# SpursLipu/YOLOv3v4-ModelCompression-MultidatasetTraining-Multibackbone

Measured on AMD Instinct MI355X. Metric: images/sec YOLOv3-608 train fp16, higher is better.
Workload: dtype f16; 1 GPU; YOLOv3 Darknet-53 608 COCO (80 classes) fp16 training step, batch 64/GPU: train-mode forward (batch-stat BN) + compute_loss + backward + nesterov SGD, single GPU; global_batch=64, parallelism=dp1

## Files before the change

include/yolo_hip.h:

```cpp
#ifndef YOLO_HIP_H
#define YOLO_HIP_H

#include <stdint.h>

#ifdef __cplusplus
extern "C" {
#endif

#define YH_ABI_VERSION 2

enum { YH_F16 = 0, YH_F32 = 1, YH_I8 = 2 };

enum { YH_ACT_LINEAR = 0, YH_ACT_LEAKY = 1, YH_ACT_RELU = 2, YH_ACT_RELU6 = 3, YH_ACT_HSWISH = 4, YH_ACT_MISH = 5 };

enum {
    YH_OK = 0,
    YH_EINVAL = -1,
    YH_EALIGN = -2,
    YH_EUNSUPPORTED = -3,
    YH_ENOMEM = -4,
    YH_ERANGE = -5
};

int yh_abi_version(void);
// ... 24 lines not shown
    float acc_scale;
    float out_scale;
    int32_t y_h, y_w;
    int32_t y_off_h, y_off_w;
    float* stats_ws;
    int64_t stats_ws_floats;
    float q_rx, q_ra, q_scale_x, q_scale_a, q_inv_scale_sum;
    const void* bwd_z;
    const float* bwd_gamma;
    const float* bwd_beta;
    const float* bwd_mean;
    const float* bwd_invstd;
    int32_t bwd_ldz, bwd_act;
    float bwd_slope;
    int32_t bwd_reserved;
} yh_conv_desc;
int64_t yh_conv2d_stats_rows(const yh_conv_desc* d);
int64_t yh_conv2d_bwd_stats_rows(const yh_conv_desc* d);

int yh_conv2d_fwd(const yh_conv_desc* d, void* stream);
int yh_qconv_pack_weights(const float* q_weight, float w_scale, const int32_t* cin_map, int cout, int cin, int kh, int kw,
                          int cin_k, int m_pad, void* packed, void* stream);
int yh_conv2d_tile(const yh_conv_desc* d);

typedef struct yh_stem_desc {
    const float* x;
    const float* w;
    const float* bias;
    void* y;
    int32_t n, cin, h, w_in, ho, wo, cout, cout_pad, kh, kw, stride, pad, ldy, act;
    float slope;
    int32_t dtype;
    float out_scale;
// ... 356 lines not shown
```

yolov3v4-modelcompression-multidatasettraining-multibackbone_amd/csrc/conv_igemm.h:

```cpp
#pragma once
#include <type_traits>

#include "common.h"

namespace yh {

struct ConvArgs {
    const void* x;
    const void* w;
    const float* bias;
    const void* res;
    void* y;
    int N, H, W, Cin, Ho, Wo, Cout, R, S, stride, pad;
    int ldx, ldr, ldy;
    int cin_k;
    int ktot;
    long P;
    int m_tiles, p_tiles;
    int m_pad;
    float acc_scale, out_scale, inv_out_scale;
    int act;
    float slope;
    int ups;
    float* stats_part;
    int y_h, y_w, y_off_h, y_off_w;
    float q_rx, q_ra, q_scale_x, q_scale_a, q_inv_scale_sum;
    int no_lds_store;
    int hpp_stagger;
    const void* bz;
    const float *bgamma, *bbeta, *bmean, *binvstd;
    int ldbz, bact;
    float bslope;
};

template <int CTRL> __device__ __forceinline__ float dpp_shr_add(float v) {
    const int t = __builtin_amdgcn_update_dpp(0, __builtin_bit_cast(int, v), CTRL, 0xf, 0xf, true);
    return v + __builtin_bit_cast(float, t);
}
__device__ __forceinline__ float row16_sum(float v) {
    v = dpp_shr_add<0x111>(v);
    v = dpp_shr_add<0x112>(v);
    v = dpp_shr_add<0x114>(v);
    v = dpp_shr_add<0x118>(v);
    return v;
}

template <int N, typename F> __device__ __forceinline__ void static_for(F&& f) {
// ... 422 lines not shown
                if (a.ups == 2) {
                    store4<OutT>(dst + a.ldy, v[0], v[1], v[2], v[3]);
                    store4<OutT>(dst + (long)c.wo2 * a.ldy, v[0], v[1], v[2], v[3]);
                    store4<OutT>(dst + (long)(c.wo2 + 1) * a.ldy, v[0], v[1], v[2], v[3]);
                }
            }
        });
    });
}

int launch_k64_tile(const ConvArgs& a, int tile, int dtype, int out_f32, hipStream_t stream);
int launch_pointwise_tile(const ConvArgs& a, int dtype, int out_f32, hipStream_t stream);
int launch_stream3_tile(const ConvArgs& a, int dtype, hipStream_t stream);
long stream3_stats_rows(long P, int cout);
int launch_pwl_tile(const ConvArgs& a, int dtype, hipStream_t stream);
bool pwl_supported(int dtype, int out_f32, int cin, int cin_k, int cout, long P, int ldx, int ldy, int ldr, const void* x, const void* y,
                   const void* res, bool stats, bool bwd);
long pwl_stats_rows(long P, int cout, bool bwd = false);
int launch_hpp_tile(const ConvArgs& a, int dtype, hipStream_t stream);
bool hpp_geometry(int W, int cin_k, int bk, int* rows_hp, int* lb, int* hbufs, size_t* lds);

}
```

yolov3v4-modelcompression-multidatasettraining-multibackbone_amd/csrc/conv_igemm.hip:

```cpp
#include "conv_igemm.h"

namespace yh {

template <typename T, int TM, int TN, int KU> struct MmaStep;

template <int TM, int TN, int KU> struct MmaStep<f16, TM, TN, KU> {
    static __device__ __forceinline__ void run(const u32x4* As, const u32x4* Bs, int BM, int BN, int arow, int brow,
                                               int lane, f32x4 (&acc)[TM][TN]) {
        const int r = lane & 15;
#pragma unroll
        for (int h = 0; h < KU / 4; ++h) {
            const int u = h * 4 + (lane >> 4);
            f16x8 a[TM], b[TN];
#pragma unroll
            for (int i = 0; i < TM; ++i) {
                u32x4 v = As[u * BM + arow + i * 16 + r];
                a[i] = *reinterpret_cast<f16x8*>(&v);
            }
#pragma unroll
            for (int j = 0; j < TN; ++j) {
                u32x4 v = Bs[u * BN + brow + j * 16 + r];
                b[j] = *reinterpret_cast<f16x8*>(&v);
            }
#pragma unroll
// ... 880 lines not shown

static bool pwl_desc_supported(const yh_conv_desc* d) {
    if (d->kh != 1 || d->kw != 1 || d->stride != 1 || d->pad != 0 || d->ups != 1) return false;
    if (d->act != YH_ACT_LINEAR && d->act != YH_ACT_LEAKY && d->act != YH_ACT_MISH) return false;
    const bool bwd = d->bwd_z != nullptr;
    if (bwd && (d->act != YH_ACT_LINEAR || (d->bwd_act != YH_ACT_LEAKY && d->bwd_act != YH_ACT_MISH))) return false;
    return yh::pwl_supported(d->dtype, d->out_f32, d->cin, d->cin_k, d->cout, (long)d->n * d->ho * d->wo, d->ldx, d->ldy, d->ldr, d->x, d->y,
                             d->res, !bwd && d->stats_ws != nullptr, bwd);
}
static bool pick_pwl_tile(const yh_conv_desc* d) {
    static const bool off = getenv("YH_NO_PWL") != nullptr;
    static const long min_px = [] { const char* e = getenv("YH_PWL_MIN_PIXELS"); return e ? atol(e) : 262144L; }();
    return !off && pwl_desc_supported(d) && (long)d->n * d->ho * d->wo >= min_px;
}

extern "C" int yh_conv2d_tile(const yh_conv_desc* d) {
    if (!d) return YH_EINVAL;
    if (d->tile != 0) return d->tile;
    if (pick_pointwise_tile(d)) return 71;
    if (pick_pwl_tile(d)) return 73;
    if (pick_stream3_tile(d)) return 72;
    if (pick_hpp_tile(d)) return 43;
    if (pick_halo_tile(d)) return 41;
    if (const int pp = pick_pp_tile(d)) return pp;
    const int t = yh::pick_tile(d->cout, (long)d->n * d->ho * d->wo, d->cin_k, d->dtype == YH_F16 ? 8 : 4, d->kh * d->kw);
    if (d->ups == 2 && (t == 21 || t == 26 || t == 27 || t == 25)) {
        if (d->dtype == YH_F16) return 24;
        if (d->dtype == YH_I8) return 25;
    }
    if (d->dtype == YH_I8 && (t == 21 || t == 27) && (long)d->cin_k * d->kh * d->kw <= 256) return 25;
    return (d->dtype == YH_I8 && t == 3) ? 24 : t;
}
// ... 94 lines not shown
    a.P = (long)d->n * d->ho * d->wo;
    a.m_tiles = a.p_tiles = 0;
    a.m_pad = d->m_pad;
    a.acc_scale = d->acc_scale; a.out_scale = d->out_scale; a.inv_out_scale = d->out_scale > 0.f ? 1.f / d->out_scale : 0.f;
    a.act = d->act; a.slope = d->slope; a.ups = d->ups;
    a.y_h = d->y_h; a.y_w = d->y_w; a.y_off_h = d->y_off_h; a.y_off_w = d->y_off_w;
    a.q_rx = d->q_rx; a.q_ra = d->q_ra; a.q_scale_x = d->q_scale_x; a.q_scale_a = d->q_scale_a; a.q_inv_scale_sum = d->q_inv_scale_sum;
    if (d->dtype == YH_I8 && d->res) qadd_pow2_args(a);
    a.no_lds_store = getenv("YH_PW_DIRECT") != nullptr;
    a.hpp_stagger = 0;
    a.stats_part = nullptr;
    a.bz = nullptr;
    a.bgamma = a.bbeta = a.bmean = a.binvstd = nullptr;
    a.ldbz = a.bact = 0;
    a.bslope = 0.f;
    if (d->bwd_z) {
        const int64_t rows = yh_conv2d_bwd_stats_rows(d);
        if (rows <= 0) return YH_EUNSUPPORTED;
        if (!d->stats_ws || d->stats_ws_floats < rows * 2 * d->cout) return YH_EINVAL;
        a.stats_part = d->stats_ws;
        a.bz = d->bwd_z; a.ldbz = d->bwd_ldz; a.bact = d->bwd_act; a.bslope = d->bwd_slope;
        a.bgamma = d->bwd_gamma; a.bbeta = d->bwd_beta; a.bmean = d->bwd_mean; a.binvstd = d->bwd_invstd;
        return launch_pwl_tile(a, d->dtype, (hipStream_t)stream);
    }
    if (d->stats_ws) {
        if (d->ups != 1 || d->res || d->dtype == YH_I8 || (d->tile >= 40 && d->tile < 50 && d->tile != 43)) return YH_EINVAL;
        const int64_t rows = yh_conv2d_stats_rows(d);
        if (rows <= 0 || d->stats_ws_floats < rows * 2 * d->cout) return YH_EINVAL;
        a.stats_part = d->stats_ws;
    }
// ... 28 lines not shown
```

yolov3v4-modelcompression-multidatasettraining-multibackbone_amd/csrc/conv_pw_lds.hip:

```cpp
#include "conv_igemm.h"

namespace yh {

template <typename T> struct PwlMma;
template <> struct PwlMma<f16> {
    typedef f16x8 frag_t;
    typedef f32x4 acc_t;
    static __device__ __forceinline__ acc_t mma(const frag_t& a, const frag_t& b, const acc_t& c) {
        return __builtin_amdgcn_mfma_f32_16x16x32_f16(a, b, c, 0, 0, 0);
    }
};
template <> struct PwlMma<int8_t> {
    typedef i32x4 frag_t;
    typedef i32x4 acc_t;
    static __device__ __forceinline__ acc_t mma(const frag_t& a, const frag_t& b, const acc_t& c) {
        return __builtin_amdgcn_mfma_i32_16x16x64_i8(a, b, c, 0, 0, 0);
    }
};

template <typename T, int MT, int KS, int MS, int ACT, int MODE>
__global__ __launch_bounds__(512, 2) void conv1x1_lds_kernel(const ConvArgs a, const int nblocks) {
    typedef typename PwlMma<T>::frag_t frag_t;
    typedef typename PwlMma<T>::acc_t acc_t;
    static_assert(sizeof(T) == 2 || MODE == 0, "int8: plain mode only");
    constexpr bool RES = MODE == 1 || MODE == 3, BWD = MODE == 3 || MODE == 4;
    constexpr int CACT = BWD ? YH_ACT_LINEAR : ACT;
    constexpr int ES = sizeof(T), VEC = 16 / ES, KB = 4 * VEC;
    constexpr int NW = 8, TN = 2, BP = TN * 16;
    constexpr int ROWB = MT * 16 * ES;
    constexpr int PITCH = ROWB + 16;
    constexpr int UNITS = ROWB / 16;
    constexpr int RPI = 64 / UNITS;
    constexpr int NPASS = BP / RPI;
    constexpr int W_BYTES = MS * MT * KS * 1024;
    constexpr int BIAS_BYTES = MS * MT * 16 * 4;
    extern __shared__ __attribute__((aligned(16))) unsigned char pl_smem[];
    unsigned char* const wl = pl_smem;
    float* const bl = reinterpret_cast<float*>(pl_smem + W_BYTES);
    const int tid = threadIdx.x, lane = tid & 63;
    const int wave = __builtin_amdgcn_readfirstlane(tid >> 6);
    unsigned char* const tile = pl_smem + W_BYTES + BIAS_BYTES + wave * (BP * PITCH);
    const int pc = lane & 15, kq = lane >> 4, mq = kq << 2;
    const T* const xg = reinterpret_cast<const T*>(a.x);
    const T* const rg = reinterpret_cast<const T*>(a.res);
    T* const yg = reinterpret_cast<T*>(a.y);

    {
        const T* const wg = reinterpret_cast<const T*>(a.w);
        for (int f = wave; f < MS * MT * KS; f += NW) {
            const int rgp = f / KS, k = f - rgp * KS;
            const u32x4 v = *reinterpret_cast<const u32x4*>(wg + (long)(rgp * 16 + pc) * a.cin_k + k * KB + kq * VEC);
            *reinterpret_cast<u32x4*>(wl + (f * 64 + lane) * 16) = v;
        }
        for (int m = tid; m < MS * MT * 16; m += NW * 64) bl[m] = m < a.Cout ? a.bias[m] : 0.f;
    }
    __syncthreads();

    const int half = wave % MS;
    const int stream = (blockIdx.x * NW + wave) / MS, nstreams = gridDim.x * NW / MS;
    const int ch0 = half * MT * 16;
    const unsigned char* const wl_h = wl + half * (MT * KS * 1024) + lane * 16;
    const float* const bl_h = bl + ch0 + mq;

    const int cu = lane % UNITS, rr = lane / UNITS;
    float s1[8], s2[8];
#pragma unroll
    for (int e = 0; e < 8; ++e) s1[e] = s2[e] = 0.f;
    float pg[8], pb[8], pm[8], pi[8];
    const T* const zg = reinterpret_cast<const T*>(a.bz);
    if constexpr (BWD) {
#pragma unroll
        for (int e = 0; e < 8; ++e) {
            const int c = ch0 + cu * 8 + e;
            pg[e] = a.bgamma[c];
            pb[e] = a.bbeta[c];
            pm[e] = a.bmean[c];
            pi[e] = a.binvstd[c];
        }
    }

    frag_t fb[TN][KS];
    u32x4 rv[NPASS];
    u32x4 zv[BWD ? NPASS : 1];
    auto load_z = [&](int blk) {
#pragma unroll
        for (int q = 0; q < (BWD ? NPASS : 0); ++q) {
            long p = (long)blk * BP + rr + q * RPI;
            p = p < a.P ? p : a.P - 1;
            zv[q] = *reinterpret_cast<const u32x4*>(zg + p * a.ldbz + ch0 + cu * VEC);
        }
    };
    auto load_b = [&](int blk, int k) {
#pragma unroll
        for (int j = 0; j < TN; ++j) {
            long p = (long)blk * BP + j * 16 + pc;
            p = p < a.P ? p : a.P - 1;
            fb[j][k] = *reinterpret_cast<const frag_t*>(xg + p * a.ldx + k * KB + kq * VEC);
        }
    };
    auto load_res = [&](int blk) {
#pragma unroll
        for (int q = 0; q < NPASS; ++q) {
            long p = (long)blk * BP + rr + q * RPI;
            p = p < a.P ? p : a.P - 1;
            rv[q] = *reinterpret_cast<const u32x4*>(rg + p * a.ldr + ch0 + cu * VEC);
        }
    };

    int blk = stream;
    if (blk < nblocks) {
#pragma unroll
        for (int k = 0; k < KS; ++k) load_b(blk, k);
        if constexpr (RES) load_res(blk);
    }
    for (; blk < nblocks; blk += nstreams) {
        const int nb = blk + nstreams < nblocks ? blk + nstreams : blk;
        if constexpr (BWD) load_z(blk);
        if constexpr (RES) {
#pragma unroll
            for (int q = 0; q < NPASS; ++q) *reinterpret_cast<u32x4*>(tile + (rr + q * RPI) * PITCH + cu * 16) = rv[q];
        }
        acc_t acc[MT][TN];
#pragma unroll
        for (int i = 0; i < MT; ++i)
#pragma unroll
            for (int j = 0; j < TN; ++j) acc[i][j] = acc_t{0, 0, 0, 0};
#pragma unroll
        for (int k = 0; k < KS; ++k) {
            frag_t wa[MT];
#pragma unroll
            for (int i = 0; i < MT; ++i) wa[i] = *reinterpret_cast<const frag_t*>(wl_h + (i * KS + k) * 1024);
#pragma unroll
            for (int i = 0; i < MT; ++i)
#pragma unroll
                for (int j = 0; j < TN; ++j) acc[i][j] = PwlMma<T>::mma(wa[i], fb[j][k], acc[i][j]);
            load_b(nb, k);
        }
        if constexpr (RES) load_res(nb);
        __builtin_amdgcn_wave_barrier();
#pragma unroll
        for (int i = 0; i < MT; ++i) {
            const f32x4 bv = *reinterpret_cast<const f32x4*>(bl_h + i * 16);
#pragma unroll
            for (int j = 0; j < TN; ++j) {
                T* const cell = reinterpret_cast<T*>(tile + (j * 16 + pc) * PITCH) + i * 16 + mq;
                float v[4];
                if constexpr (sizeof(T) == 1) {
                    quantize4<CACT>(acc[i][j], bv, a, v);
                } else {
#pragma unroll
                    for (int e = 0; e < 4; ++e) v[e] = activate_t<CACT, T>(acc[i][j][e] + bv[e], a.slope);
// ... 42 lines not shown
        for (int e = 0; e < 8; ++e)
#pragma unroll
            for (int m = UNITS; m < 64; m <<= 1) {
                s1[e] += __shfl_xor(s1[e], m);
                s2[e] += __shfl_xor(s2[e], m);
            }
        if (lane < UNITS) {
            float* const row = a.stats_part + (long)stream * 2 * a.Cout + ch0 + cu * 8;
#pragma unroll
            for (int e = 0; e < 8; ++e) {
                row[e] = s1[e];
                row[a.Cout + e] = s2[e];
            }
        }
    }
}

static bool pwl_shape(int cin_k, int cout, int kb, int* mt, int* ks, int* ms, bool bwd = false) {
    if (cin_k % kb || cout % 16 || cout < 32 || cout > 256 || cin_k < kb || cin_k > 8 * kb) return false;
    *ms = bwd ? cout / 64 : (cout > 128 ? 2 : 1);
    if (bwd && (cout % 64 || *ms < 1)) return false;
    if (cout % (16 * *ms)) return false;
    *mt = cout / (16 * *ms);
    *ks = cin_k / kb;
    if (*mt > 8 || (*mt != 2 && *mt != 4 && *mt != 8) || (*ks != 1 && *ks != 2 && *ks != 4 && *ks != 8)) return false;
    return (long)cout * cin_k * (kb == 32 ? 2 : 1) <= 64 * 1024;
}

static int pwl_ms(int cout, bool bwd) { return bwd ? cout / 64 : (cout > 128 ? 2 : 1); }

// ... 39 lines not shown
    return (long)pwl_grid(P, ms, &nblocks) * 8 / ms;
}

template <typename T, int MT, int KS, int MS, int ACT> static int launch_pwl_mode(const ConvArgs& a, hipStream_t s) {
    int nblocks;
    const int grid = pwl_grid(a.P, MS, &nblocks);
    const size_t lds = (size_t)MS * MT * KS * 1024 + (size_t)MS * MT * 16 * 4 + (size_t)8 * 32 * (MT * 16 * sizeof(T) + 16);
#define YH_PWL_GO(MODE)                                                                                       \
    do {                                                                                                      \
        auto kern = conv1x1_lds_kernel<T, MT, KS, MS, ACT, MODE>;                                             \
        const hipError_t e = ensure_dynamic_lds(reinterpret_cast<const void*>(kern), lds);                    \
        if (e != hipSuccess) return (int)e;                                                                   \
        hipLaunchKernelGGL(kern, dim3(grid), dim3(512), lds, s, a, nblocks);                                  \
    } while (0)
    if constexpr (sizeof(T) == 1) {
        if (a.stats_part || a.res || a.bz) return YH_EUNSUPPORTED;
        YH_PWL_GO(0);
    } else {
        if (a.bz) {
            if constexpr ((ACT == YH_ACT_LEAKY || ACT == YH_ACT_MISH) && MT == 4 && ((KS == 1 && MS == 1) || (KS == 2 && MS == 2) || (KS == 4 && MS == 4))) {
                if (!a.stats_part) return YH_EINVAL;
                if (a.res) YH_PWL_GO(3);
                else YH_PWL_GO(4);
            } else {
                return YH_EUNSUPPORTED;
            }
        } else if (a.stats_part) YH_PWL_GO(2);
        else if (a.res) YH_PWL_GO(1);
        else YH_PWL_GO(0);
    }
#undef YH_PWL_GO
    return check_launch();
}

template <typename T, int MT, int KS, int MS> static int launch_pwl_act(const ConvArgs& a, hipStream_t s) {
    switch (a.bz ? a.bact : a.act) {
        case YH_ACT_LINEAR: return launch_pwl_mode<T, MT, KS, MS, YH_ACT_LINEAR>(a, s);
        case YH_ACT_LEAKY: return launch_pwl_mode<T, MT, KS, MS, YH_ACT_LEAKY>(a, s);
        case YH_ACT_MISH: return launch_pwl_mode<T, MT, KS, MS, YH_ACT_MISH>(a, s);
        default: return YH_EUNSUPPORTED;
    }
}

int launch_pwl_tile(const ConvArgs& a, int dtype, hipStream_t s) {
    int mt, ks, ms;
    if (!pwl_shape(a.cin_k, a.Cout, dtype == YH_I8 ? 64 : 32, &mt, &ks, &ms, a.bz != nullptr)) return YH_EUNSUPPORTED;
#define YH_PWL_CASE(T, M, K, S2) if (mt == M && ks == K && ms == S2) return launch_pwl_act<T, M, K, S2>(a, s)
    if (dtype == YH_I8) {
        YH_PWL_CASE(int8_t, 8, 4, 1);
        YH_PWL_CASE(int8_t, 4, 2, 1);
        YH_PWL_CASE(int8_t, 8, 2, 1);
        YH_PWL_CASE(int8_t, 4, 1, 1);
        YH_PWL_CASE(int8_t, 8, 4, 2);
        YH_PWL_CASE(int8_t, 8, 2, 2);
        return YH_EUNSUPPORTED;
    }
    if (dtype != YH_F16) return YH_EUNSUPPORTED;
    YH_PWL_CASE(f16, 2, 2, 1);
    YH_PWL_CASE(f16, 4, 1, 1);
    YH_PWL_CASE(f16, 4, 4, 1);
    YH_PWL_CASE(f16, 8, 2, 1);
    YH_PWL_CASE(f16, 8, 8, 1);
    YH_PWL_CASE(f16, 8, 4, 2);
    YH_PWL_CASE(f16, 8, 4, 1);
    YH_PWL_CASE(f16, 4, 2, 1);
    YH_PWL_CASE(f16, 4, 2, 2);
    YH_PWL_CASE(f16, 4, 4, 4);
#undef YH_PWL_CASE
    return YH_EUNSUPPORTED;
}

}
// ... 1 lines not shown
```

yolov3v4-modelcompression-multidatasettraining-multibackbone_amd/engine/hiplib.py:

```python
import ctypes as C
import os

_HERE = os.path.dirname(os.path.abspath(__file__))
LIB_PATH = os.environ.get('YOLO_HIP_LIB') or os.path.join(os.path.dirname(_HERE), 'libyolo_hip.so')

YH_F16, YH_F32, YH_I8 = 0, 1, 2
ACT_CODES = {'linear': 0, 'leaky': 1, 'relu': 2, 'relu6': 3, 'h_swish': 4, 'mish': 5}
OP_CONV, OP_STEM, OP_POOL, OP_COPY, OP_ADD, OP_DECODE, OP_DW, OP_SE, OP_QCOPY, OP_QPOOL, OP_QADD = 1, 2, 3, 4, 5, 6, 7, 8, 9, 10, 11

_i32, _f32, _vp, _i64 = C.c_int32, C.c_float, C.c_void_p, C.c_int64


class ConvDesc(C.Structure):
    _fields_ = [('x', _vp), ('w', _vp), ('bias', _vp), ('res', _vp), ('y', _vp),
                ('n', _i32), ('h', _i32), ('w_in', _i32), ('cin', _i32),
                ('ho', _i32), ('wo', _i32), ('cout', _i32),
                ('kh', _i32), ('kw', _i32), ('stride', _i32), ('pad', _i32),
                ('ldx', _i32), ('ldr', _i32), ('ldy', _i32),
                ('cin_k', _i32), ('m_pad', _i32),
                ('act', _i32), ('slope', _f32), ('ups', _i32), ('out_f32', _i32), ('dtype', _i32), ('tile', _i32),
                ('acc_scale', _f32), ('out_scale', _f32),
                ('y_h', _i32), ('y_w', _i32), ('y_off_h', _i32), ('y_off_w', _i32), ('stats_ws', _vp), ('stats_ws_floats', _i64),
                ('q_rx', _f32), ('q_ra', _f32), ('q_scale_x', _f32), ('q_scale_a', _f32), ('q_inv_scale_sum', _f32),
                ('bwd_z', _vp), ('bwd_gamma', _vp), ('bwd_beta', _vp), ('bwd_mean', _vp), ('bwd_invstd', _vp),
                ('bwd_ldz', _i32), ('bwd_act', _i32), ('bwd_slope', _f32), ('bwd_reserved', _i32)]


class StemDesc(C.Structure):
    _fields_ = [('x', _vp), ('w', _vp), ('bias', _vp), ('y', _vp),
                ('n', _i32), ('cin', _i32), ('h', _i32), ('w_in', _i32), ('ho', _i32), ('wo', _i32),
                ('cout', _i32), ('cout_pad', _i32), ('kh', _i32), ('kw', _i32), ('stride', _i32), ('pad', _i32),
                ('ldy', _i32), ('act', _i32), ('slope', _f32), ('dtype', _i32), ('out_scale', _f32),
                ('stats_ws', _vp), ('stats_ws_floats', _i64)]


class PoolDesc(C.Structure):
    _fields_ = [('x', _vp), ('y', _vp),
                ('n', _i32), ('h', _i32), ('w_in', _i32), ('c', _i32), ('ho', _i32), ('wo', _i32), ('k', _i32),
                ('stride', _i32), ('pad_lo', _i32), ('edge_zero', _i32), ('ldx', _i32), ('ldy', _i32), ('dtype', _i32)]

# ... 205 lines not shown
           BnBwdReduceDesc: OP_BN_BWD_REDUCE, BnBwdApplyDesc: OP_BN_BWD_APPLY, WgradDesc: OP_WGRAD,
           StemWgradDesc: OP_STEM_WGRAD, DilateDesc: OP_DILATE2, UpsampleBwdDesc: OP_UPSAMPLE2_BWD, CastDesc: OP_CAST_F32, LayoutDesc: OP_NCHW_TO_NHWC, PoolBwdDesc: OP_POOL_BWD, PackBatchDesc: OP_PACK_BATCH, DwWgradDesc: OP_DW_WGRAD, DwDgradDesc: OP_DW_DGRAD,
           SeBwdDesc: OP_SE_BWD, StemBwdDesc: OP_STEM_BWD,
           ConvDesc: OP_CONV, StemDesc: OP_STEM, PoolDesc: OP_POOL, CopyDesc: OP_COPY, AddDesc: OP_ADD,
           DecodeDesc: OP_DECODE, DwDesc: OP_DW, SeDesc: OP_SE, QCopyDesc: OP_QCOPY, QPoolDesc: OP_QPOOL, QAddDesc: OP_QADD}

_SIGNATURES = {
    'yh_abi_version': (C.c_int, []),
    'yh_error_string': (C.c_char_p, [C.c_int]),
    'yh_conv_pack_weights': (C.c_int, [C.c_int, _vp, _vp, _vp, _vp, _vp, _vp, _f32, _vp, C.c_int, C.c_int, C.c_int,
                                       C.c_int, C.c_int, C.c_int, _vp, _vp, _vp]),
    'yh_conv2d_fwd': (C.c_int, [C.POINTER(ConvDesc), _vp]),
    'yh_conv2d_tile': (C.c_int, [C.POINTER(ConvDesc)]),
    'yh_conv2d_stats_rows': (_i64, [C.POINTER(ConvDesc)]),
    'yh_conv2d_bwd_stats_rows': (_i64, [C.POINTER(ConvDesc)]),
    'yh_plan_set_async_reduce': (C.c_int, [_vp, C.c_int]),
    'yh_qconv_pack_weights': (C.c_int, [_vp, _f32, _vp, C.c_int, C.c_int, C.c_int, C.c_int, C.c_int, C.c_int, _vp, _vp]),
    'yh_stem_pack_weights': (C.c_int, [_vp, _vp, _vp, _vp, _vp, _vp, _f32, C.c_int, C.c_int, C.c_int, C.c_int, C.c_int,
                                       _vp, _vp, _vp]),
    'yh_conv2d_stem_fwd': (C.c_int, [C.POINTER(StemDesc), _vp]),
    'yh_conv2d_stem_stats_rows': (_i64, [C.POINTER(StemDesc)]),
    'yh_qmish_selftest': (C.c_int, [C.c_uint32, C.c_uint32, _f32, _vp, _vp]),
    'yh_dw_pack_weights': (C.c_int, [C.c_int, _vp, _vp, _vp, _vp, _vp, _vp, _f32, _vp, C.c_int, C.c_int, C.c_int, _vp, _vp, _vp]),
    'yh_dwconv2d_fwd': (C.c_int, [C.POINTER(DwDesc), _vp]),
    'yh_se_fwd': (C.c_int, [C.POINTER(SeDesc), _vp]),
    'yh_maxpool2d_fwd': (C.c_int, [C.POINTER(PoolDesc), _vp]),
    'yh_qcopy': (C.c_int, [C.POINTER(QCopyDesc), _vp]),
    'yh_qpool': (C.c_int, [C.POINTER(PoolDesc), _vp]),
    'yh_qadd': (C.c_int, [C.POINTER(QAddDesc), _vp]),
    'yh_copy_channels': (C.c_int, [C.POINTER(CopyDesc), _vp]),
# ... 125 lines not shown
```

yolov3v4-modelcompression-multidatasettraining-multibackbone_amd/engine/train.py:

```python
import ctypes as C
import os

import torch
import torch.nn as nn

from . import hiplib
from .hiplib import (ConvDesc, StemDesc, CopyDesc, AddDesc, BnStatsDesc, BnFinalizeDesc, BnActFwdDesc, BnBwdReduceDesc,
                     BnBwdApplyDesc, WgradDesc, StemWgradDesc, StemBwdDesc, UpsampleBwdDesc, CastDesc, LayoutDesc, PoolDesc, PoolBwdDesc, PackItem, PackBatchDesc, DwDesc, SeDesc, DwWgradDesc,
                     DwDgradDesc, SeBwdDesc, BnL1Row)
from .plan import DarknetEngine, ALIGN_C, _round_up

_FUSED_DGRAD_MAX_CIN = int(os.environ.get('YOLO_HIP_FUSED_DGRAD_MAX', '64'))

SLOT_INPUT = 0
SLOT_WS = 1
SLOT_WS2 = 63
SLOT_HEAD0 = 2
LINEAR = hiplib.ACT_CODES['linear']


class ChannelAlignmentError(NotImplementedError):
    """The aligned lowering wants every tensor width to be a multiple of 8: ``engine/padded.py`` trains such graphs through a
    channel-padded twin."""

# ... 237 lines not shown
            if v.kind in ('qadd',):
                raise NotImplementedError('HIP training path: %s blocks are not lowered yet (block %s)' % (v.kind, v.block))
            if v.kind == 'conv':
                if v.src.kind != 'input' and (v.src.C % ALIGN_C or v.src.c_phys != v.src.C):
                    raise ChannelAlignmentError('HIP training path: channel counts must be multiples of %d' % ALIGN_C)
                if not v.fp32 and v.C % ALIGN_C:
                    raise ChannelAlignmentError('HIP training path: channel counts must be multiples of %d' % ALIGN_C)
                if v.src.kind == 'input' and (v.src.C > 4 or v.src.C > ALIGN_C):
                    raise NotImplementedError('HIP training path: the first conv reads at most 4 image channels')
                if v.stride == 2 and not (v.k == 3 and v.pad == 1):
                    raise NotImplementedError('HIP training path: stride-2 convs must be 3x3 pad 1')
                if v.stride not in (1, 2):
                    raise NotImplementedError('HIP training path: conv stride %d' % v.stride)
                if v.bn is not None and v.fp32:
                    raise NotImplementedError('HIP training path: BatchNorm on a yolo-head conv')

    def _build_train_plan(self, N, Cin, H, W):
        values, heads, outs = self._build_values(N, Cin, H, W)
        self._check_supported(values)
        self._place(values)
        lib, dev, P = self.lib, self.device, hiplib.ptr
        plan = dict(values=values, heads=heads, N=N, storages=[], fwd_ops=[], bwd_ops=[], zero_list=[], ws_floats=0, ws2_floats=0,
                    arena=self._arena, arena_refs=[], state=_PlanState(dev), bound=None)
        fwd = plan['fwd'] = lib.yh_plan_create()
        bwd = plan['bwd'] = lib.yh_plan_create()
        if not fwd or not bwd:
            raise MemoryError('yh_plan_create failed')
        stats = plan['stats'] = _Arena()
        saved = plan['saved'] = _Arena()
        grads = plan['grads'] = _Arena()
# ... 171 lines not shown
                hiplib.check(lib.yh_plan_add_dep(bwd, op, r), 'yh_plan_add_dep')
                dz_state['reader'][k] = None

        def on_side_lane(op, k):
            if not two_lanes:
                return
            hiplib.check(lib.yh_plan_set_lane(bwd, op, 1), 'yh_plan_set_lane')
            hiplib.check(lib.yh_plan_add_dep(bwd, op, op - 1), 'yh_plan_add_dep')
            dz_state['reader'][k] = op
        head_index = {id(h.src): k for k, h in enumerate(heads)}

        raw, n_items = self._pack_items(plan)
        plan['pack_table'] = keep(len(raw), torch.uint8, zero=True)
        add(fwd, plan['fwd_ops'], PackBatchDesc(items=plan['pack_table'].data_ptr(), n_items=n_items), 'pack')

        for v in values:
            if v.kind == 'input':
                continue
            y = None if v.storage is None else P(v.storage, v.c_off)
            if v.kind == 'conv':
                pk, s = v.tpack, v.src
                fused_stats = 0
                direct = v.plain
                zt = None if direct else v.z
                if s.kind == 'input':
                    d = StemDesc(x=None, w=P(pk['w']), bias=P(pk['b']), y=y if direct else P(zt), n=N, cin=s.C, h=s.H,
                                 w_in=s.W, ho=v.Ho, wo=v.Wo, cout=v.c_phys, cout_pad=pk['cout_pad'], kh=v.k, kw=v.k,
                                 stride=v.stride, pad=v.pad, ldy=v.ld if direct else v.c_phys, act=LINEAR, slope=0.0,
                                 dtype=self.code, out_scale=0.0)
                    if v.c_phys > pk['cout_pad'] or v.fp32:
# ... 2 lines not shown
                        fused_stats = int(lib.yh_conv2d_stem_stats_rows(C.byref(d)))
                        if fused_stats:
                            d.stats_ws_floats = fused_stats * 2 * v.c_phys
                            plan['ws_floats'] = max(plan['ws_floats'], d.stats_ws_floats)
                    op = add(fwd, plan['fwd_ops'], d, 'stem%d' % v.block)
                    fixup(fwd, op, StemDesc, 'x', SLOT_INPUT)
                    if fused_stats:
                        fixup(fwd, op, StemDesc, 'stats_ws', SLOT_WS)
                else:
                    d = ConvDesc(x=P(s.storage, s.c_off), w=P(pk['w']), bias=P(pk['b']), res=None,
                                 y=None if v.fp32 else (y if direct else P(zt)), n=N, h=s.H, w_in=s.W, cin=s.c_phys,
                                 ho=v.Ho, wo=v.Wo, cout=v.c_phys, kh=v.k, kw=v.k, stride=v.stride, pad=v.pad, ldx=s.ld,
                                 ldr=0, ldy=v.c_phys if (v.fp32 or not direct) else v.ld, cin_k=pk['cin_k'],
                                 m_pad=pk['m_pad'], act=LINEAR, slope=0.0, ups=1, out_f32=1 if v.fp32 else 0,
                                 dtype=self.code, tile=self.force_tile, acc_scale=0.0, out_scale=0.0)
                    if v.bn is not None and not direct:
                        fused_stats = int(lib.yh_conv2d_stats_rows(C.byref(d)))
                        if fused_stats:
                            d.stats_ws_floats = fused_stats * 2 * v.c_phys
                            plan['ws_floats'] = max(plan['ws_floats'], d.stats_ws_floats)
                    op = add(fwd, plan['fwd_ops'], d, 'conv%d' % v.block)
                    if fused_stats:
                        fixup(fwd, op, ConvDesc, 'stats_ws', SLOT_WS)
                    if v.fp32:
                        fixup(fwd, op, ConvDesc, 'y', SLOT_HEAD0 + head_index[id(v)])
                if direct:
                    continue
                pixels = N * v.Ho * v.Wo
                bn = v.bn
                base = dict(z=P(zt), pixels=pixels, n=N, h=v.Ho, w_in=v.Wo, c=v.c_phys, ldz=v.c_phys, act=v.act,
# ... 6 lines not shown
                        raise NotImplementedError('HIP training path: BatchNorm without momentum / running stats / affine')
                    for t in (bn.weight, bn.bias, bn.running_mean, bn.running_var):
                        if t.dtype != torch.float32 or not t.is_contiguous():
                            raise NotImplementedError('HIP training path: BatchNorm tensors must be contiguous fp32')
                    fused = bool(fused_stats)
                    if not fused:
                        add_reduction(fwd, plan['fwd_ops'], BnStatsDesc(**base, **bnp), 'bnstat%d' % v.block)
                    fin = BnFinalizeDesc(**base, **bnp, running_mean=P(bn.running_mean), running_var=P(bn.running_var),
                                         nparts=fused_stats if fused else 0, ws_floats=(fused_stats * 2 * v.c_phys) if fused else 0)
                    op = add(fwd, plan['fwd_ops'], fin, 'bnfin%d' % v.block)
                    if fused:
                        fixup(fwd, op, BnFinalizeDesc, 'ws', SLOT_WS)
                else:
                    bnp = dict()
                v.bn_args = (base, bnp)
                add(fwd, plan['fwd_ops'],
                    BnActFwdDesc(**base, **bnp, out=y, ldo=v.ld, res=None if v.res is None else P(v.res.storage, v.res.c_off),
                                 ldr=0 if v.res is None else v.res.ld), 'bnact%d' % v.block)
            elif v.kind == 'dw':
                s, pk, bn = v.src, v.tpack, v.bn
                zt = None if v.plain else v.z
                add(fwd, plan['fwd_ops'],
                    DwDesc(x=P(s.storage, s.c_off), w=P(pk['w']), bias=P(pk['b']), y=y if v.plain else P(zt), n=N, h=s.H, w_in=s.W,
                           c=s.c_phys, ho=v.H, wo=v.W, k=v.k, stride=v.stride, pad=v.pad, ldx=s.ld, ldy=v.ld if v.plain else v.c_phys,
                           act=LINEAR, slope=0.0, dtype=self.code), 'dw%d' % v.block)
                if not v.plain:
                    pixels = N * v.H * v.W
                    base = dict(z=P(zt), pixels=pixels, n=N, h=v.H, w_in=v.W, c=v.c_phys, ldz=v.c_phys, act=v.act, slope=v.slope,
                                dtype=self.code, ups=1)
                    bnp = dict()
# ... 542 lines not shown
```

Measured before the change: 1259 images/s.

## Fuse producer BN+activation(+residual) into following 1x1 pointwise conv prologue

Adds a pre-op path to the LDS pointwise conv kernel that takes the raw pre-BN output z of the previous conv, applies batch-norm, activation and an optional residual add in registers, writes the activated tensor out for later consumers, and feeds it straight into the MMA. The planner detects conv->1x1 conv pairs where the 1x1 conv is the first reader and skips the separate bnact kernel for them. This removes one full read and a kernel launch for each fused activation tensor. In exchange the kernel carries more registers and LDS for the BN table and the residual prefetch, and the planner now has to check reader order.

```diff
diff --git a/include/yolo_hip.h b/include/yolo_hip.h
--- a/include/yolo_hip.h
+++ b/include/yolo_hip.h
@@ -62,9 +62,20 @@
     int32_t bwd_ldz, bwd_act;
     float bwd_slope;
     int32_t bwd_reserved;
+    const void* pre_z;
+    const void* pre_res;
+    void* pre_y;
+    const float* pre_gamma;
+    const float* pre_beta;
+    const float* pre_mean;
+    const float* pre_invstd;
+    int32_t pre_ldz, pre_ldr, pre_ldy, pre_act;
+    float pre_slope;
+    int32_t pre_reserved;
 } yh_conv_desc;
 int64_t yh_conv2d_stats_rows(const yh_conv_desc* d);
 int64_t yh_conv2d_bwd_stats_rows(const yh_conv_desc* d);
+int yh_conv2d_pre_bn_ok(const yh_conv_desc* d);
 
 int yh_conv2d_fwd(const yh_conv_desc* d, void* stream);
 int yh_qconv_pack_weights(const float* q_weight, float w_scale, const int32_t* cin_map, int cout, int cin, int kh, int kw,
diff --git a/yolov3v4-modelcompression-multidatasettraining-multibackbone_amd/csrc/conv_igemm.h b/yolov3v4-modelcompression-multidatasettraining-multibackbone_amd/csrc/conv_igemm.h
--- a/yolov3v4-modelcompression-multidatasettraining-multibackbone_amd/csrc/conv_igemm.h
+++ b/yolov3v4-modelcompression-multidatasettraining-multibackbone_amd/csrc/conv_igemm.h
@@ -31,6 +31,11 @@
     const float *bgamma, *bbeta, *bmean, *binvstd;
     int ldbz, bact;
     float bslope;
+    const void *pz, *pres;
+    void* py;
+    const float *pgamma, *pbeta, *pmean, *pinvstd;
+    int ldpz, ldpr, ldpy, pact;
+    float pslope;
 };
 
 template <int CTRL> __device__ __forceinline__ float dpp_shr_add(float v) {
@@ -483,6 +488,7 @@
 int launch_stream3_tile(const ConvArgs& a, int dtype, hipStream_t stream);
 long stream3_stats_rows(long P, int cout);
 int launch_pwl_tile(const ConvArgs& a, int dtype, hipStream_t stream);
+bool pwl_pre_supported(int cin_k, int cout, int pact, int ldpz, int ldpr, int ldpy, const void* pz, const void* pres, const void* py);
 bool pwl_supported(int dtype, int out_f32, int cin, int cin_k, int cout, long P, int ldx, int ldy, int ldr, const void* x, const void* y,
                    const void* res, bool stats, bool bwd);
 long pwl_stats_rows(long P, int cout, bool bwd = false);
diff --git a/yolov3v4-modelcompression-multidatasettraining-multibackbone_amd/csrc/conv_igemm.hip b/yolov3v4-modelcompression-multidatasettraining-multibackbone_amd/csrc/conv_igemm.hip
--- a/yolov3v4-modelcompression-multidatasettraining-multibackbone_amd/csrc/conv_igemm.hip
+++ b/yolov3v4-modelcompression-multidatasettraining-multibackbone_amd/csrc/conv_igemm.hip
@@ -918,8 +918,19 @@
     return !off && pwl_desc_supported(d) && (long)d->n * d->ho * d->wo >= min_px;
 }
 
+static bool pre_bn_ok(const yh_conv_desc* d) {
+    if (!d || !d->pre_z || !d->pre_y || !d->pre_gamma || !d->pre_beta || !d->pre_mean || !d->pre_invstd) return false;
+    if (d->n <= 0 || d->ho <= 0 || d->wo <= 0 || d->dtype != YH_F16 || d->out_f32 || d->act != YH_ACT_LINEAR || d->res || d->bwd_z) return false;
+    if (d->x != d->pre_y || d->ldx != d->pre_ldy || d->pre_z == d->pre_y) return false;
+    if (d->tile != 0 && d->tile != 73) return false;
+    if (!yh::pwl_pre_supported(d->cin_k, d->cout, d->pre_act, d->pre_ldz, d->pre_ldr, d->pre_ldy, d->pre_z, d->pre_res, d->pre_y)) return false;
+    return d->tile == 73 ? pwl_desc_supported(d) : pick_pwl_tile(d);
+}
+extern "C" int yh_conv2d_pre_bn_ok(const yh_conv_desc* d) { return pre_bn_ok(d) ? 1 : 0; }
+
 extern "C" int yh_conv2d_tile(const yh_conv_desc* d) {
     if (!d) return YH_EINVAL;
+    if (d->pre_z) return pre_bn_ok(d) ? 73 : YH_EUNSUPPORTED;
     if (d->tile != 0) return d->tile;
     if (pick_pointwise_tile(d)) return 71;
     if (pick_pwl_tile(d)) return 73;
@@ -1044,6 +1055,18 @@
     a.bgamma = a.bbeta = a.bmean = a.binvstd = nullptr;
     a.ldbz = a.bact = 0;
     a.bslope = 0.f;
+    a.pz = a.pres = nullptr;
+    a.py = nullptr;
+    a.pgamma = a.pbeta = a.pmean = a.pinvstd = nullptr;
+    a.ldpz = a.ldpr = a.ldpy = a.pact = 0;
+    a.pslope = 0.f;
+    if (d->pre_z) {
+        if (!pre_bn_ok(d)) return YH_EUNSUPPORTED;
+        a.pz = d->pre_z; a.pres = d->pre_res; a.py = d->pre_y;
+        a.ldpz = d->pre_ldz; a.ldpr = d->pre_res ? d->pre_ldr : 0; a.ldpy = d->pre_ldy;
+        a.pgamma = d->pre_gamma; a.pbeta = d->pre_beta; a.pmean = d->pre_mean; a.pinvstd = d->pre_invstd;
+        a.pact = d->pre_act; a.pslope = d->pre_slope;
+    }
     if (d->bwd_z) {
         const int64_t rows = yh_conv2d_bwd_stats_rows(d);
         if (rows <= 0) return YH_EUNSUPPORTED;
diff --git a/yolov3v4-modelcompression-multidatasettraining-multibackbone_amd/csrc/conv_pw_lds.hip b/yolov3v4-modelcompression-multidatasettraining-multibackbone_amd/csrc/conv_pw_lds.hip
--- a/yolov3v4-modelcompression-multidatasettraining-multibackbone_amd/csrc/conv_pw_lds.hip
+++ b/yolov3v4-modelcompression-multidatasettraining-multibackbone_amd/csrc/conv_pw_lds.hip
@@ -18,11 +18,16 @@
     }
 };
 
-template <typename T, int MT, int KS, int MS, int ACT, int MODE>
-__global__ __launch_bounds__(512, 2) void conv1x1_lds_kernel(const ConvArgs a, const int nblocks) {
+template <typename T, int MT, int KS, int MS, int ACT, int MODE, int PACT, bool PRES>
+__device__ __forceinline__ void conv1x1_lds_body(const ConvArgs& a, const int nblocks) {
     typedef typename PwlMma<T>::frag_t frag_t;
     typedef typename PwlMma<T>::acc_t acc_t;
     static_assert(sizeof(T) == 2 || MODE == 0, "int8: plain mode only");
+    constexpr bool PRE = PACT >= 0;
+    static_assert(!PRE || (sizeof(T) == 2 && MS == 1 && (MODE == 0 || MODE == 2)), "pre-op: fp16, one wave per pixel stream, plain / statistics");
+    constexpr int PD = KS < 4 ? KS : (MT * KS == 64 ? 2 : 4);
+    constexpr int ZD = PRE ? (KS < 4 ? KS : 4) : KS;
+    constexpr int PT_BYTES = PRE ? KS * 4 * 32 * 4 : 0;
     constexpr bool RES = MODE == 1 || MODE == 3, BWD = MODE == 3 || MODE == 4;
     constexpr int CACT = BWD ? YH_ACT_LINEAR : ACT;
     constexpr int ES = sizeof(T), VEC = 16 / ES, KB = 4 * VEC;
@@ -39,9 +44,13 @@
     float* const bl = reinterpret_cast<float*>(pl_smem + W_BYTES);
     const int tid = threadIdx.x, lane = tid & 63;
     const int wave = __builtin_amdgcn_readfirstlane(tid >> 6);
-    unsigned char* const tile = pl_smem + W_BYTES + BIAS_BYTES + wave * (BP * PITCH);
+    unsigned char* const tile = pl_smem + W_BYTES + BIAS_BYTES + PT_BYTES + wave * (BP * PITCH);
+    float* const ptab = reinterpret_cast<float*>(pl_smem + W_BYTES + BIAS_BYTES);
     const int pc = lane & 15, kq = lane >> 4, mq = kq << 2;
-    const T* const xg = reinterpret_cast<const T*>(a.x);
+    const T* const xg = reinterpret_cast<const T*>(PRE ? a.pz : a.x);
+    const int ldxg = PRE ? a.ldpz : a.ldx;
+    const T* const prg = reinterpret_cast<const T*>(a.pres);
+    T* const pyg = reinterpret_cast<T*>(a.py);
     const T* const rg = reinterpret_cast<const T*>(a.res);
     T* const yg = reinterpret_cast<T*>(a.y);
 
@@ -53,6 +62,15 @@
             *reinterpret_cast<u32x4*>(wl + (f * 64 + lane) * 16) = v;
         }
         for (int m = tid; m < MS * MT * 16; m += NW * 64) bl[m] = m < a.Cout ? a.bias[m] : 0.f;
+        if constexpr (PRE) {
+            for (int c = tid; c < KS * KB; c += NW * 64) {
+                float* const row = ptab + (c >> 3) * 32 + (c & 7);
+                row[0] = a.pgamma[c];
+                row[8] = a.pbeta[c];
+                row[16] = a.pmean[c];
+                row[24] = a.pinvstd[c];
+            }
+        }
     }
     __syncthreads();
 
@@ -79,7 +97,8 @@
         }
     }
 
-    frag_t fb[TN][KS];
+    frag_t fb[TN][ZD];
+    frag_t pr[PRE && PRES ? PD : 1][TN];
     u32x4 rv[NPASS];
     u32x4 zv[BWD ? NPASS : 1];
     auto load_z = [&](int blk) {
@@ -95,7 +114,15 @@
         for (int j = 0; j < TN; ++j) {
             long p = (long)blk * BP + j * 16 + pc;
             p = p < a.P ? p : a.P - 1;
-            fb[j][k] = *reinterpret_cast<const frag_t*>(xg + p * a.ldx + k * KB + kq * VEC);
+            fb[j][k % ZD] = *reinterpret_cast<const frag_t*>(xg + p * ldxg + k * KB + kq * VEC);
+        }
+    };
+    auto load_pres = [&](int blk, int k, int slot) {
+#pragma unroll
+        for (int j = 0; j < TN; ++j) {
+            long p = (long)blk * BP + j * 16 + pc;
+            p = p < a.P ? p : a.P - 1;
+            pr[slot][j] = *reinterpret_cast<const frag_t*>(prg + p * a.ldpr + k * KB + kq * VEC);
         }
     };
     auto load_res = [&](int blk) {
@@ -110,8 +137,12 @@
     int blk = stream;
     if (blk < nblocks) {
 #pragma unroll
-        for (int k = 0; k < KS; ++k) load_b(blk, k);
+        for (int k = 0; k < ZD; ++k) load_b(blk, k);
         if constexpr (RES) load_res(blk);
+        if constexpr (PRE && PRES) {
+#pragma unroll
+            for (int k = 0; k < PD; ++k) load_pres(blk, k, k);
+        }
     }
     for (; blk < nblocks; blk += nstreams) {
         const int nb = blk + nstreams < nblocks ? blk + nstreams : blk;
@@ -127,14 +158,53 @@
             for (int j = 0; j < TN; ++j) acc[i][j] = acc_t{0, 0, 0, 0};
 #pragma unroll
         for (int k = 0; k < KS; ++k) {
+            if constexpr (PRE) {
+                const float* const pp = ptab + (k * 4 + kq) * 32;
+                float ga[8], be[8], mu[8], is[8];
+#pragma unroll
+                for (int h = 0; h < 2; ++h) {
+                    const f32x4 g4 = *reinterpret_cast<const f32x4*>(pp + h * 4), b4 = *reinterpret_cast<const f32x4*>(pp + 8 + h * 4);
+                    const f32x4 m4 = *reinterpret_cast<const f32x4*>(pp + 16 + h * 4), i4 = *reinterpret_cast<const f32x4*>(pp + 24 + h * 4);
+#pragma unroll
+                    for (int e = 0; e < 4; ++e) {
+                        ga[h * 4 + e] = g4[e];
+                        be[h * 4 + e] = b4[e];
+                        mu[h * 4 + e] = m4[e];
+                        is[h * 4 + e] = i4[e];
+                    }
+                }
+#pragma unroll
+                for (int j = 0; j < TN; ++j) {
+                    const frag_t v = fb[j][k % ZD];
+                    float o[8];
+#pragma unroll
+                    for (int e = 0; e < 8; ++e) o[e] = activate_train_t<T>(ga[e] * (((float)v[e] - mu[e]) * is[e]) + be[e], PACT, a.pslope);
+                    if constexpr (PRES) {
+                        const frag_t r = pr[k % PD][j];
+#pragma unroll
+                        for (int e = 0; e < 8; ++e) o[e] += (float)r[e];
+                    }
+                    frag_t ov;
+#pragma unroll
+                    for (int e = 0; e < 8; ++e) ov[e] = (T)o[e];
+                    fb[j][k % ZD] = ov;
+                    const long p = (long)blk * BP + j * 16 + pc;
+                    if (p < a.P) *reinterpret_cast<frag_t*>(pyg + p * a.ldpy + k * KB + kq * VEC) = ov;
+                }
+                if constexpr (PRES) {
+                    if (k + PD < KS) load_pres(blk, k + PD, k % PD);
+                    else load_pres(nb, k + PD - KS, k % PD);
+                }
+            }
             frag_t wa[MT];
 #pragma unroll
             for (int i = 0; i < MT; ++i) wa[i] = *reinterpret_cast<const frag_t*>(wl_h + (i * KS + k) * 1024);
 #pragma unroll
             for (int i = 0; i < MT; ++i)
 #pragma unroll
-                for (int j = 0; j < TN; ++j) acc[i][j] = PwlMma<T>::mma(wa[i], fb[j][k], acc[i][j]);
-            load_b(nb, k);
+                for (int j = 0; j < TN; ++j) acc[i][j] = PwlMma<T>::mma(wa[i], fb[j][k % ZD], acc[i][j]);
+            if (k + ZD < KS) load_b(blk, k + ZD);
+            else load_b(nb, k + ZD - KS);
         }
         if constexpr (RES) load_res(nb);
         __builtin_amdgcn_wave_barrier();
@@ -207,6 +277,15 @@
             }
         }
     }
+}
+
+template <typename T, int MT, int KS, int MS, int ACT, int MODE>
+__global__ __launch_bounds__(512, 2) void conv1x1_lds_kernel(const ConvArgs a, const int nblocks) {
+    conv1x1_lds_body<T, MT, KS, MS, ACT, MODE, -1, false>(a, nblocks);
+}
+template <int MT, int KS, int MODE, int PACT, bool PRES>
+__global__ __launch_bounds__(512, 2) void conv1x1_lds_pre_kernel(const ConvArgs a, const int nblocks) {
+    conv1x1_lds_body<f16, MT, KS, 1, YH_ACT_LINEAR, MODE, PACT, PRES>(a, nblocks);
 }
 
 static bool pwl_shape(int cin_k, int cout, int kb, int* mt, int* ks, int* ms, bool bwd = false) {
@@ -276,7 +355,7 @@
         hipLaunchKernelGGL(kern, dim3(grid), dim3(512), lds, s, a, nblocks);                                  \
     } while (0)
     if constexpr (sizeof(T) == 1) {
-        if (a.stats_part || a.res || a.bz) return YH_EUNSUPPORTED;
+        if (a.stats_part || a.res || a.bz || a.pz) return YH_EUNSUPPORTED;
         YH_PWL_GO(0);
     } else {
         if (a.bz) {
@@ -292,6 +371,56 @@
         else YH_PWL_GO(0);
     }
 #undef YH_PWL_GO
+    return check_launch();
+}
+
+static bool pwl_pre_case(int mt, int ks, int ms) {
+    return ms == 1 && ((mt == 2 && ks == 2) || (mt == 4 && ks == 4) || (mt == 8 && ks == 8));
+}
+
+bool pwl_pre_supported(int cin_k, int cout, int pact, int ldpz, int ldpr, int ldpy, const void* pz, const void* pres, const void* py) {
+    int mt, ks, ms;
+    if (!pwl_shape(cin_k, cout, 32, &mt, &ks, &ms) || !pwl_pre_case(mt, ks, ms)) return false;
+    if (pact != YH_ACT_LEAKY && pact != YH_ACT_MISH) return false;
+    if (pact == YH_ACT_MISH && pres && mt == 8 && ks == 8) return false;
+    return ldpz % 8 == 0 && ldpy % 8 == 0 && (!pres || ldpr % 8 == 0) && ldpz >= cin_k && ldpy >= cin_k && (!pres || ldpr >= cin_k) &&
+           aligned16(pz) && aligned16(py) && (!pres || aligned16(pres));
+}
+
+template <int MT, int KS> static int launch_pwl_pre(const ConvArgs& a, hipStream_t s) {
+    int nblocks;
+    const int grid = pwl_grid(a.P, 1, &nblocks);
+    const size_t lds = (size_t)MT * KS * 1024 + (size_t)MT * 16 * 4 + (size_t)KS * 512 + (size_t)8 * 32 * (MT * 16 * sizeof(f16) + 16);
+#define YH_PWL_PRE_GO(MODE, PACT, PRES)                                                                       \
+    do {                                                                                                      \
+        auto kern = conv1x1_lds_pre_kernel<MT, KS, MODE, PACT, PRES>;                                         \
+        const hipError_t e = ensure_dynamic_lds(reinterpret_cast<const void*>(kern), lds);                    \
+        if (e != hipSuccess) return (int)e;                                                                   \
+        hipLaunchKernelGGL(kern, dim3(grid), dim3(512), lds, s, a, nblocks);                                  \
+    } while (0)
+#define YH_PWL_PRE_RES(MODE, PACT)                                                                            \
+    do {                                                                                                      \
+        if (a.pres) YH_PWL_PRE_GO(MODE, PACT, true);                                                          \
+        else YH_PWL_PRE_GO(MODE, PACT, false);                                                                \
+    } while (0)
+    if (a.res || a.bz || a.act != YH_ACT_LINEAR) return YH_EUNSUPPORTED;
+    if (a.pact == YH_ACT_LEAKY) {
+        if (a.stats_part) YH_PWL_PRE_RES(2, YH_ACT_LEAKY);
+        else YH_PWL_PRE_RES(0, YH_ACT_LEAKY);
+    } else if (a.pact == YH_ACT_MISH) {
+        if constexpr (MT == 8 && KS == 8) {
+            if (a.pres) return YH_EUNSUPPORTED;
+            if (a.stats_part) YH_PWL_PRE_GO(2, YH_ACT_MISH, false);
+            else YH_PWL_PRE_GO(0, YH_ACT_MISH, false);
+        } else {
+            if (a.stats_part) YH_PWL_PRE_RES(2, YH_ACT_MISH);
+            else YH_PWL_PRE_RES(0, YH_ACT_MISH);
+        }
+    } else {
+        return YH_EUNSUPPORTED;
+    }
+#undef YH_PWL_PRE_RES
+#undef YH_PWL_PRE_GO
     return check_launch();
 }
 
@@ -318,6 +447,12 @@
         return YH_EUNSUPPORTED;
     }
     if (dtype != YH_F16) return YH_EUNSUPPORTED;
+    if (a.pz) {
+        if (mt == 2 && ks == 2 && ms == 1) return launch_pwl_pre<2, 2>(a, s);
+        if (mt == 4 && ks == 4 && ms == 1) return launch_pwl_pre<4, 4>(a, s);
+        if (mt == 8 && ks == 8 && ms == 1) return launch_pwl_pre<8, 8>(a, s);
+        return YH_EUNSUPPORTED;
+    }
     YH_PWL_CASE(f16, 2, 2, 1);
     YH_PWL_CASE(f16, 4, 1, 1);
     YH_PWL_CASE(f16, 4, 4, 1);
diff --git a/yolov3v4-modelcompression-multidatasettraining-multibackbone_amd/engine/hiplib.py b/yolov3v4-modelcompression-multidatasettraining-multibackbone_amd/engine/hiplib.py
--- a/yolov3v4-modelcompression-multidatasettraining-multibackbone_amd/engine/hiplib.py
+++ b/yolov3v4-modelcompression-multidatasettraining-multibackbone_amd/engine/hiplib.py
@@ -23,7 +23,10 @@
                 ('y_h', _i32), ('y_w', _i32), ('y_off_h', _i32), ('y_off_w', _i32), ('stats_ws', _vp), ('stats_ws_floats', _i64),
                 ('q_rx', _f32), ('q_ra', _f32), ('q_scale_x', _f32), ('q_scale_a', _f32), ('q_inv_scale_sum', _f32),
                 ('bwd_z', _vp), ('bwd_gamma', _vp), ('bwd_beta', _vp), ('bwd_mean', _vp), ('bwd_invstd', _vp),
-                ('bwd_ldz', _i32), ('bwd_act', _i32), ('bwd_slope', _f32), ('bwd_reserved', _i32)]
+                ('bwd_ldz', _i32), ('bwd_act', _i32), ('bwd_slope', _f32), ('bwd_reserved', _i32),
+                ('pre_z', _vp), ('pre_res', _vp), ('pre_y', _vp), ('pre_gamma', _vp), ('pre_beta', _vp), ('pre_mean', _vp),
+                ('pre_invstd', _vp), ('pre_ldz', _i32), ('pre_ldr', _i32), ('pre_ldy', _i32), ('pre_act', _i32),
+                ('pre_slope', _f32), ('pre_reserved', _i32)]
 
 
 class StemDesc(C.Structure):
@@ -259,6 +262,7 @@
     'yh_conv2d_tile': (C.c_int, [C.POINTER(ConvDesc)]),
     'yh_conv2d_stats_rows': (_i64, [C.POINTER(ConvDesc)]),
     'yh_conv2d_bwd_stats_rows': (_i64, [C.POINTER(ConvDesc)]),
+    'yh_conv2d_pre_bn_ok': (C.c_int, [C.POINTER(ConvDesc)]),
     'yh_plan_set_async_reduce': (C.c_int, [_vp, C.c_int]),
     'yh_qconv_pack_weights': (C.c_int, [_vp, _f32, _vp, C.c_int, C.c_int, C.c_int, C.c_int, C.c_int, C.c_int, _vp, _vp]),
     'yh_stem_pack_weights': (C.c_int, [_vp, _vp, _vp, _vp, _vp, _vp, _f32, C.c_int, C.c_int, C.c_int, C.c_int, C.c_int,
diff --git a/yolov3v4-modelcompression-multidatasettraining-multibackbone_amd/engine/train.py b/yolov3v4-modelcompression-multidatasettraining-multibackbone_amd/engine/train.py
--- a/yolov3v4-modelcompression-multidatasettraining-multibackbone_amd/engine/train.py
+++ b/yolov3v4-modelcompression-multidatasettraining-multibackbone_amd/engine/train.py
@@ -275,6 +275,78 @@
                     raise NotImplementedError('HIP training path: conv stride %d' % v.stride)
                 if v.bn is not None and v.fp32:
                     raise NotImplementedError('HIP training path: BatchNorm on a yolo-head conv')
+
+    @staticmethod
+    def _value_refs(u):
+        refs = [getattr(u, 'src', None), getattr(u, 'res', None), getattr(u, 'a', None), getattr(u, 'b', None)]
+        refs += list(getattr(u, 'srcs', None) or [])
+        refs += [part[0] for part in getattr(u, 'parts', None) or []]
+        return [r for r in refs if r is not None]
+
+    def _pre_bn_desc(self, L, P, N):
+        def ld_of(v):
+            if v.ld is not None:
+                return v.ld
+            if v.parent is not None:
+                return ld_of(v.parent)
+            return ld_of(v.src) if v.kind == 'slice' else v.c_phys
+
+        probe = {}
+
+        def at(t, c_off=0):
+            if isinstance(t, int):
+                return t
+            if getattr(t, 'storage', None) is not None:
+                return hiplib.ptr(t.storage, t.c_off)
+            base = probe.setdefault(id(t), (len(probe) + 1) << 24)
+            return base + 2 * c_off
+        z = getattr(P, 'z', None)
+        bn = P.bn
+        state = getattr(P, 'bn_args', None)
+        if state is not None:
+            gamma, beta, mean, invstd = (state[1][k] for k in ('gamma', 'beta', 'mean', 'invstd'))
+        else:
+            gamma, beta, mean, invstd = at(bn.weight.data_ptr() or 16), at(bn.bias.data_ptr() or 16), 16, 16
+        y = at(P, P.c_off)
+        pk = getattr(L, 'tpack', None) or dict(cin_k=_round_up(P.c_phys, self.kstep), m_pad=_round_up(L.c_phys, 128), w=None, b=None)
+        return ConvDesc(x=y, w=hiplib.ptr(pk['w']), bias=hiplib.ptr(pk['b']), res=None, y=None, n=N, h=P.H, w_in=P.W, cin=P.c_phys,
+                        ho=L.Ho, wo=L.Wo, cout=L.c_phys, kh=1, kw=1, stride=1, pad=0, ldx=ld_of(P), ldr=0, ldy=L.c_phys,
+                        cin_k=pk['cin_k'], m_pad=pk['m_pad'], act=LINEAR, slope=0.0, ups=1, out_f32=0, dtype=self.code,
+                        tile=self.force_tile, acc_scale=0.0, out_scale=0.0,
+                        pre_z=hiplib.ptr(z) if z is not None else (len(probe) + 64) << 24,
+                        pre_res=None if P.res is None else at(P.res, P.res.c_off), pre_y=y, pre_gamma=gamma, pre_beta=beta,
+                        pre_mean=mean, pre_invstd=invstd, pre_ldz=P.c_phys, pre_ldr=0 if P.res is None else ld_of(P.res),
+                        pre_ldy=ld_of(P), pre_act=P.act, pre_slope=P.slope)
+
+    def _pre_bn_pairs(self, values, N):
+        query = getattr(self.lib, 'yh_conv2d_pre_bn_ok', None)
+        if query is None or self.dtype != torch.float16 or os.environ.get('YOLO_HIP_PRE_BN', '1') == '0':
+            return {}
+        first = {}
+        for u in values:
+            for r in self._value_refs(u):
+                first.setdefault(id(r), u)
+        pairs = {}
+        for P in values:
+            L = first.get(id(P))
+            if P.kind != 'conv' or L is None or L.kind != 'conv' or L.src is not P:
+                continue
+            if P.bn is None or P.fp32 or P.ups != 1 or P.parent is not None or P.src.kind == 'input' or getattr(P, 'plain', False):
+                continue
+            if L.k != 1 or L.stride != 1 or L.ups != 1 or L.fp32 or L.pad != 0:
+                continue
+            d = self._pre_bn_desc(L, P, N)
+            if int(query(C.byref(d))) == 1:
+                pairs[id(P)] = (P, L)
+        return pairs
+
+    @staticmethod
+    def _assert_first_reader(log, piece, what):
+        for name, desc in log:
+            for field, ctype in desc._fields_:
+                val = getattr(desc, field) if ctype is C.c_void_p else None
+                if val and val >> 62 == 1 and (val ^ _PIECE_TAG) >> _PIECE_SHIFT == piece:
+                    raise AssertionError('%s forms its input itself, but %s (field %s) uses that buffer before it' % (what, name, field))
 
     def _build_train_plan(self, N, Cin, H, W):
         values, heads, outs = self._build_values(N, Cin, H, W)
@@ -476,6 +548,9 @@
         plan['pack_table'] = keep(len(raw), torch.uint8, zero=True)
         add(fwd, plan['fwd_ops'], PackBatchDesc(items=plan['pack_table'].data_ptr(), n_items=n_items), 'pack')
 
+        pre_bn = self._pre_bn_pairs(values, N)
+        pre_bn_of = {id(L): Pv for Pv, L in pre_bn.values()}
+        plan['pre_bn'] = sorted(L.block for _, L in pre_bn.values())
         for v in values:
             if v.kind == 'input':
                 continue
@@ -508,6 +583,14 @@
                                  ldr=0, ldy=v.c_phys if (v.fp32 or not direct) else v.ld, cin_k=pk['cin_k'],
                                  m_pad=pk['m_pad'], act=LINEAR, slope=0.0, ups=1, out_f32=1 if v.fp32 else 0,
                                  dtype=self.code, tile=self.force_tile, acc_scale=0.0, out_scale=0.0)
+                    if id(v) in pre_bn_of:
+                        q = self._pre_bn_desc(v, s, N)
+                        for name, _ in ConvDesc._fields_:
+                            if name.startswith('pre_'):
+                                setattr(d, name, getattr(q, name))
+                        if int(lib.yh_conv2d_pre_bn_ok(C.byref(d))) != 1:
+                            raise RuntimeError('conv%d: the library withdrew the pre-op form it offered' % v.block)
+                        self._assert_first_reader(plan['fwd_ops'][s.pre_bn_from:], s.storage.index, 'conv%d' % v.block)
                     if v.bn is not None and not direct:
                         fused_stats = int(lib.yh_conv2d_stats_rows(C.byref(d)))
                         if fused_stats:
@@ -544,6 +627,9 @@
                 else:
                     bnp = dict()
                 v.bn_args = (base, bnp)
+                if id(v) in pre_bn:
+                    v.pre_bn_from = len(plan['fwd_ops'])
+                    continue
                 add(fwd, plan['fwd_ops'],
                     BnActFwdDesc(**base, **bnp, out=y, ldo=v.ld, res=None if v.res is None else P(v.res.storage, v.res.c_off),
                                  ldr=0 if v.res is None else v.res.ld), 'bnact%d' % v.block)
```

Result: slower. 1241 images/s (-1.4%).
